# Jarvis73/PEMP

Measured on AMD Instinct MI355X. Metric: episodes/sec (PEMP stage-1 eval step, PASCAL-5i-shaped 1-shot, ResNet-50), higher is better.
Workload: dtype f32

## Files before the change

pemp_amd/csrc/conv_stem_pool.hip:

```cpp
#include "conv_common.h"

namespace pemp {

typedef __attribute__((address_space(3))) void* lptr_t;

namespace {
constexpr int SP_PH = 8, SP_PW = 8;
constexpr int SP_CH = 2 * SP_PH + 1, SP_CW = 2 * SP_PW + 1;
constexpr int SP_IH = 2 * (SP_CH - 1) + 7, SP_IW = 2 * (SP_CW - 1) + 7;
constexpr int SP_ROWS = SP_CH * SP_CW;
constexpr int SP_NW = (SP_ROWS + 31) / 32;
constexpr int SP_TAPS = 49, SP_NK = 7;
constexpr int SP_XQ = SP_IH * SP_IW;
constexpr int SP_XI = (SP_XQ + 63) / 64;
constexpr int SP_BQ = 64 * 12;
constexpr int SP_LDS_OPS = (SP_XI * 64 + 2 * SP_BQ) * 16, SP_LDS_EPI = SP_ROWS * 64 * 4;
constexpr int SP_LDS = SP_LDS_OPS > SP_LDS_EPI ? SP_LDS_OPS : SP_LDS_EPI;
static_assert(SP_NW * 64 <= 1024 && SP_LDS <= 80 * 1024, "two blocks per CU");

__host__ __device__ constexpr int sp_tap_off(int tap) { return (tap / 7) * SP_IW + tap % 7; }
}

__global__ __launch_bounds__(SP_NW * 64) void conv_stem_pool_kernel(ConvArgs a, int Hp, int Wp, int nph, int npw) {
#if defined(__HIP_DEVICE_COMPILE__)
    extern __shared__ __attribute__((aligned(16))) v4f smem[];
    v4f* Xs = smem;
    v4f* Bs = smem + SP_XI * 64;

    const int tid = threadIdx.x;
    const int lane = tid & 63;
    const int wave = __builtin_amdgcn_readfirstlane(tid >> 6);
    const int lr = lane & 31, lh = lane >> 5;

    const int ntn = a.Cout / 64;
    int t = xcd_tile_order(blockIdx.x, gridDim.x);
    const int n0 = (t % ntn) * 64;
    t /= ntn;
    const int pxb = t % npw;
    t /= npw;
    const int pyb = t % nph, img = t / nph;
    const int ph0 = pyb * SP_PH, pw0 = pxb * SP_PW;
    const int cy0 = 2 * ph0 - 1, cx0 = 2 * pw0 - 1;
    const int iy0 = 2 * cy0 - 3, ix0 = 2 * cx0 - 3;

    const __amdgpu_buffer_rsrc_t rx =
        __builtin_amdgcn_make_buffer_rsrc((void*)(a.x + (size_t)img * a.H * a.W * 4), 0, 0x80000000u, 0x00020000);
    const __amdgpu_buffer_rsrc_t rw = __builtin_amdgcn_make_buffer_rsrc((void*)a.w, 0, 0x80000000u, 0x00020000);

    for (int i = wave; i < SP_XI; i += SP_NW) {
        const int q = i * 64 + lane;
        const int py = q / SP_IW, px = q - py * SP_IW;
        const int iy = iy0 + py, ix = ix0 + px;
        const bool ok = q < SP_XQ && (unsigned)iy < (unsigned)a.H && (unsigned)ix < (unsigned)a.W;
        const unsigned vo = ok ? (unsigned)(iy * a.W + ix) * 16u : 0x80000000u;
        __builtin_amdgcn_raw_ptr_buffer_load_lds(rx, (lptr_t)(Xs + i * 64), 16, vo, 0, 0, 0);
    }
#define PEMP_SP_DMA_B(kt_, buf_)                                                                                  \
    for (int i = wave; i < SP_BQ / 64; i += SP_NW) {                                                              \
        const int q = i * 64 + lane, row = q / 12, pos = q - row * 12;                                            \
        const int src = PEMP_SPLIT3_SWZ(row, pos);                                                                \
        const unsigned vo = (unsigned)((n0 + row) * a.Kpad * 6 + src * 16);                                       \
        __builtin_amdgcn_raw_ptr_buffer_load_lds(rw, (lptr_t)(Bs + (buf_) * SP_BQ + i * 64), 16, vo, (kt_) * 192, 0, 0); \
    }
    PEMP_SP_DMA_B(0, 0);

    const int m = wave * 32 + lr;
    const int mc = m < SP_ROWS ? m : 0;
    const int cy = mc / SP_CW, cx = mc - cy * SP_CW;
    const v4f* Ax = Xs + 2 * cy * SP_IW + 2 * cx;
    const v4f* Bw = Bs + lr * 12;
    const int bsw = (lr >> 2) & 3;
    const v4f zero4 = {0.f, 0.f, 0.f, 0.f};

    f32x16 acc[2];
#pragma unroll
    for (int ni = 0; ni < 2; ++ni)
#pragma unroll
        for (int e = 0; e < 16; ++e) acc[ni][e] = 0.f;

#pragma unroll
    for (int kt = 0; kt < SP_NK; ++kt) {
        asm volatile("s_waitcnt vmcnt(0)" ::: "memory");
        __syncthreads();
        if (kt + 1 < SP_NK) PEMP_SP_DMA_B(kt + 1, (kt + 1) & 1);
        const v4f* Bb = Bw + (kt & 1) * SP_BQ;
#pragma unroll
        for (int s = 0; s < 2; ++s) {
            const int tap0 = kt * 8 + s * 4;
            if (tap0 >= SP_TAPS) continue;
            const bool v00 = tap0 < SP_TAPS, v01 = tap0 + 1 < SP_TAPS, v10 = tap0 + 2 < SP_TAPS, v11 = tap0 + 3 < SP_TAPS;
            const int o00 = v00 ? sp_tap_off(tap0) : 0, o01 = v01 ? sp_tap_off(tap0 + 1) : 0;
            const int o10 = v10 ? sp_tap_off(tap0 + 2) : 0, o11 = v11 ? sp_tap_off(tap0 + 3) : 0;
            v4f x0 = Ax[lh ? o10 : o00], x1 = Ax[lh ? o11 : o01];
            if (!(lh ? v10 : v00)) x0 = zero4;
            if (!(lh ? v11 : v01)) x1 = zero4;
            bf16x8 ah, am, al;
            split3_bf16(x0, x1, ah, am, al);
            const int pb = (2 * s + lh) ^ bsw;
#pragma unroll
            for (int ni = 0; ni < 2; ++ni) {
                const bf16x8 bh = __builtin_bit_cast(bf16x8, Bb[ni * 32 * 12 + pb]);
                const bf16x8 bm = __builtin_bit_cast(bf16x8, Bb[ni * 32 * 12 + 4 + pb]);
                const bf16x8 bl = __builtin_bit_cast(bf16x8, Bb[ni * 32 * 12 + 8 + pb]);
                split3_mma6(acc[ni], ah, am, al, bh, bm, bl);
            }
        }
    }
#undef PEMP_SP_DMA_B

    __syncthreads();
    float* Cs = (float*)smem;
    const bool relu = a.flags & PEMP_CONV_RELU;
#pragma unroll
    for (int ni = 0; ni < 2; ++ni) {
        const int n = n0 + ni * 32 + lr;
        const float sc = a.scale ? a.scale[n] : 1.f, sh = a.shift ? a.shift[n] : 0.f;
#pragma unroll
        for (int e = 0; e < 16; ++e) {
            const int row = wave * 32 + (e & 3) + 8 * (e >> 2) + 4 * lh;
            float o = __builtin_fmaf(acc[ni][e], sc, sh);
            if (relu) o = fmaxf(o, 0.f);
            if (row < SP_ROWS) Cs[row * 64 + ni * 32 + lr] = o;
        }
    }
    __syncthreads();
    for (int i = tid; i < SP_PH * SP_PW * 16; i += SP_NW * 64) {
        const int c4 = i & 15, pp = i >> 4;
        const int py = pp / SP_PW, px = pp - py * SP_PW;
        const int ph = ph0 + py, pw = pw0 + px;
        if (ph >= Hp || pw >= Wp) continue;
        v4f mx = {-INFINITY, -INFINITY, -INFINITY, -INFINITY};
#pragma unroll
        for (int dy = 0; dy < 3; ++dy) {
            const int ly = 2 * py + dy;
            if ((unsigned)(cy0 + ly) >= (unsigned)a.Ho) continue;
#pragma unroll
            for (int dx = 0; dx < 3; ++dx) {
                const int lx = 2 * px + dx;
                if ((unsigned)(cx0 + lx) >= (unsigned)a.Wo) continue;
                const v4f v = *(const v4f*)(Cs + (ly * SP_CW + lx) * 64 + c4 * 4);
                mx.x = fmaxf(mx.x, v.x);
                mx.y = fmaxf(mx.y, v.y);
                mx.z = fmaxf(mx.z, v.z);
                mx.w = fmaxf(mx.w, v.w);
            }
        }
        *(v4f*)(a.y + ((size_t)(img * Hp + ph) * Wp + pw) * a.ldy + n0 + c4 * 4) = mx;
    }
#endif
}

int conv_stem_pool_out(int i) {
    int o = (i + 2 - 3 + 1) / 2 + 1;
    if ((o - 1) * 2 >= i + 1) --o;
    return o;
}

int launch_conv_stem_pool(const ConvArgs& a, hipStream_t st) {
    if (!(a.flags & PEMP_CONV_STEM4) || a.KH != 7 || a.KW != 7 || a.stride != 2 || a.pad != 3 || a.dil != 1 || a.Kpad != SP_NK * 32) {
        set_error("conv2d: POOL3S2 needs the 7x7 / stride 2 / pad 3 NHWC4 stem (Kpad %d)", SP_NK * 32);
        return -1;
    }
    if (a.res || a.padv || a.stats || a.rowmask || (a.flags & (PEMP_CONV_SHIFT_PER_IMAGE | PEMP_CONV_BF16_IO))) {
        set_error("conv2d: POOL3S2 takes no residual, padding value, per-image shift or statistics");
        return -1;
    }
    const int Hp = conv_stem_pool_out(a.Ho), Wp = conv_stem_pool_out(a.Wo);
    const int nph = cdiv(Hp, SP_PH), npw = cdiv(Wp, SP_PW);
    const long long grid = (long long)a.N * nph * npw * (a.Cout / 64);
    if ((long long)a.H * a.W * 16 >= (1ll << 31) || (long long)a.Cout * a.Kpad * 6 >= (1ll << 31) || grid >= (1ll << 31) ||
        (long long)a.N * Hp * Wp * a.ldy >= (1ll << 31)) {
        set_error("conv2d: POOL3S2 operands outside 32-bit addressing");
        return -1;
    }
    static_assert(SP_LDS > 64 * 1024, "dynamic LDS attribute");
    hipError_t e = hipFuncSetAttribute((const void*)conv_stem_pool_kernel, hipFuncAttributeMaxDynamicSharedMemorySize, SP_LDS);
    if (e != hipSuccess) {
        set_error("hipFuncSetAttribute(lds=%d): %s", SP_LDS, hipGetErrorString(e));
        return (int)e;
    }
    hipLaunchKernelGGL(conv_stem_pool_kernel, dim3((unsigned)grid), dim3(SP_NW * 64), SP_LDS, st, a, Hp, Wp, nph, npw);
    return launch_status("conv_stem_pool");
}

}
```

scratch/s3_layers_bench.py:

```python
import argparse
import hashlib
import os
import sys

import torch

sys.path.insert(0, os.path.dirname(os.path.dirname(os.path.abspath(__file__))))
from pemp_amd import ops

UNSPLIT = (43, 42, 41, 44, 46, 47, 49)
SPLIT = (52, 51, 54, 56)
PANEL = ops.SPLIT3_PANEL_TILES
PRESPLIT = ops.SPLIT3_PRESPLIT_TILES
RING = getattr(ops, "SPLIT3_RING_TILES", ())
ROW3 = ops.SPLIT3_ROW3_TILES
LAYERS = ((256, 1024, 1, 1, True, False), (512, 1024, 1, 1, False, False), (1024, 256, 1, 1, False, False),
          (256, 256, 3, 2, False, False), (128, 512, 1, 1, True, False), (1024, 512, 1, 1, False, False),
          (256, 256, 3, 2, False, True),
          (64, 256, 1, 1, True, False, 1, 101), (64, 256, 1, 1, False, False, 1, 101), (256, 512, 1, 1, False, False, 2, 101),
          (128, 128, 3, 1, False, False), (128, 128, 3, 1, False, False, 2, 101), (64, 64, 3, 1, False, False, 1, 101),
          (512, 128, 1, 1, False, False),
          (512, 256, 1, 1, False, False), (256, 256, 1, 1, False, False),
          (64, 256, 1, 1, True, False, 1, 51, 101),
          (64, 64, 3, 1, False, False, 2, 101),
          (256, 256, 3, 12, False, True))


def timed(fn, reps, n=5):
    for _ in range(2):
        fn()
    e0, e1 = torch.cuda.Event(enable_timing=True), torch.cuda.Event(enable_timing=True)
    best, worst = 1e9, 0.0
    for _ in range(reps):
        e0.record()
        for _ in range(n):
            fn()
        e1.record()
        e1.synchronize()
        us = e0.elapsed_time(e1) / n * 1e3
        best, worst = min(best, us), max(worst, us)
    return best, worst


def presplit(x):
    h = x.to(torch.bfloat16)
    r = x - h.float()
    m = r.to(torch.bfloat16)
    lo = (r - m.float()).to(torch.bfloat16)
    return torch.stack([p.reshape(*x.shape[:-1], x.shape[-1] // 32, 32) for p in (h, m, lo)], dim=-2).contiguous()


def digest(t):
    return hashlib.sha1(t.cpu().numpy().tobytes()).hexdigest()[:16]


def rs2_row(dev, N, HW, HR, cin, cout, name, keep, reps):
    g = torch.Generator().manual_seed(cin * 7 + cout * 3 + 1001)
    x = torch.randn(N * HW * HW, cin, generator=g).to(dev).view(N, HW, HW, cin)
    w = (torch.randn(cout, cin, 1, 1, generator=g) * (1.0 / cin ** 0.5)).to(dev)
    packed, kpad = ops.pack_conv_weight(w)
    packed = packed.contiguous()
    prm = ops.ConvParams(packed, None, torch.randn(cout, generator=g).to(dev), cin, cout, 1, 1, 1, 0, 1, kpad, False, True, ops.pack_split3(packed))
    res = torch.randn(N, HR, HR, cout, generator=g).to(dev)
    ref = ops.conv2d(x, prm, residual=res[:, ::2, ::2, :].contiguous(), tile=43).clone()
    out = torch.empty_like(ref)
    fl = 2.0 * N * HW * HW * cout * cin
    cells = []
    for tile in keep(ops.res_s2_tiles(prm)):
        run = lambda: ops.conv2d(x, prm, residual=res, residual_stride=2, out=out, tile=tile)
        out.zero_()
        run()
        same = torch.equal(out, ref)
        us, worst = timed(run, reps)
        cells.append(f"{tile}: {us:7.1f}..{worst:6.1f}us {fl / us / 1e6:5.1f}TF{'' if same else ' !'}")
    print(f"{name:>16} k1 d1 res1 | " + " | ".join(cells), flush=True)
    print(f"{'':>16} hash 43={digest(ref)}", flush=True)


def main():
    ap = argparse.ArgumentParser()
    ap.add_argument("--only", default="", help="cin-cout-kK[-padv]: one layer")
    ap.add_argument("--reps", type=int, default=3)
    ap.add_argument("--ids", default="", help="comma-separated tile ids: only these are timed (a counter run of one kernel)")
    ap.add_argument("--producers", action="store_true", help="with --ids: time the selected ids as producers of a pre-split output too")
    ap.add_argument("--res", type=int, choices=(0, 1), default=None, help="run the selected layers without / with a residual, whatever their row says")
    args = ap.parse_args()
    dev = torch.device("cuda:0")
    N = 50
    keep = lambda ids: tuple(t for t in ids if not args.ids or str(t) in args.ids.split(","))
    for layer in LAYERS:
        cin, cout, k, dil, has_res, padv = layer[:6]
        stride, HW = layer[6:8] if len(layer) > 6 else (1, 51)
        RS2 = layer[8] if len(layer) > 8 else 0
        has_res = has_res if args.res is None or RS2 else bool(args.res)
        M = N * HW * HW
        HO = (HW - 1) // stride + 1
        name = f"{cin}-{cout}-k{k}" + (f"-d{dil}" if k == 3 and dil > 2 else "") + ("-padv" if padv else "") + (f"-s{stride}" if stride > 1 else "") + (f"-hw{HW}-res{int(has_res)}" if HW != 51 else "") + ("-rs2" if RS2 else "")
        if args.only and name not in args.only.split(","):
            continue
        if RS2:
            rs2_row(dev, N, HW, RS2, cin, cout, name, keep, args.reps)
            continue
        g = torch.Generator().manual_seed(cin * 7 + cout * 3 + k)
        buf = torch.empty(M + 4, cin, device=dev)
        buf[:M] = torch.randn(M, cin, generator=g).to(dev)
        buf[M:] = torch.randn(cin, generator=g).to(dev)
        x, pv = buf[:M].view(N, HW, HW, cin), buf[M]
        w = (torch.randn(cout, cin, k, k, generator=g) * (1.0 / (cin * k * k) ** 0.5)).to(dev)
        packed, kpad = ops.pack_conv_weight(w)
        packed = packed.contiguous()
        prm = ops.ConvParams(packed, None, torch.randn(cout, generator=g).to(dev), cin, cout, k, k, stride, dil if k == 3 else 0, dil, kpad,
                             False, True, ops.pack_split3(packed))
        res = torch.randn(N, HO, HO, cout, generator=g).to(dev) if has_res else None
        pad_value = pv if padv else None
        out = torch.empty(N, HO, HO, cout, device=dev)
        fl = 2.0 * N * HO * HO * cout * k * k * cin
        ref = ops.conv2d(x, prm, residual=res, pad_value=pad_value, tile=43).clone()
        cells, hashes = [], [f"43={digest(ref)}"]
        panel = PANEL if k == 1 and kpad <= 256 and not padv else ()
        ring = RING if k == 1 and kpad >= 128 and not has_res and not padv and cout % 128 == 0 else ()
        for tile in keep(UNSPLIT + ring + panel + SPLIT):
            if cout % ops._tile_bn(tile):
                continue
            run = lambda: ops.conv2d(x, prm, residual=res, pad_value=pad_value, out=out, tile=tile)
            run()
            same = torch.equal(out, ref)
            if tile in SPLIT:
                hashes.append(f"{tile}=" + ("43" if same else digest(out)))
            us, worst = timed(run, args.reps)
            mark = "" if same else (" ~" if tile in SPLIT else " !")
            cells.append(f"{tile}: {us:7.1f}..{worst:6.1f}us {fl / us / 1e6:5.1f}TF{mark}")
            if tile not in SPLIT and not same:
                hashes.append(f"{tile}=MISMATCH:{digest(out)}")
        if k > 1 and cout % 128 == 0:
            sbuf = torch.zeros((M + 4) * cin * 3, dtype=torch.bfloat16, device=dev)
            sbuf[:(M + 1) * cin * 3] = presplit(buf[:M + 1]).reshape(-1)
            xs, pvs = sbuf[:M * cin * 3].view(N, HW, HW, cin // 32, 3, 32), sbuf[M * cin * 3:(M + 1) * cin * 3].view(cin // 32, 3, 32)
            row3 = ROW3 if k == 3 and stride == 1 and not has_res and not padv and ops.row3_stage_rows(HW, dil) <= ops.ROW3_STAGE_ROWS else ()
            for tile in keep(PRESPLIT + row3):
                run = lambda: ops.conv2d(xs, prm, residual=res, pad_value=pvs if padv else None, out=out, tile=tile, x_split3=True)
                out.zero_()
                run()
                same = torch.equal(out, ref)
                us, worst = timed(run, args.reps)
                cells.append(f"{tile}: {us:7.1f}..{worst:6.1f}us {fl / us / 1e6:5.1f}TF{'' if same else ' !'}")
            if not has_res:
                want = presplit(ref)
                outs = torch.empty_like(want)
                for tile in keep(PRESPLIT):
                    run = lambda: ops.conv2d(xs, prm, pad_value=pvs if padv else None, out=out, tile=tile, x_split3=True, also_split3=outs)
                    out.zero_()
                    run()
                    same = torch.equal(out, ref) and torch.equal(outs.view(torch.int16), want.view(torch.int16))
                    us, worst = timed(run, args.reps)
                    cells.append(f"{tile}+s: {us:7.1f}..{worst:6.1f}us{'' if same else ' !'}")
                del want, outs
            del sbuf, xs, pvs
        if k == 1 and not has_res:
            want = presplit(ref)
            outs = torch.empty_like(want)
            for tile in keep((43, 42, 41, 44, 46, 47, 49) + ring if not args.ids or args.producers else ()):
                if cout % ops._tile_bn(tile):
                    continue
                run = lambda: ops.conv2d(x, prm, out=outs, tile=tile, out_split3=True)
                run()
                same = torch.equal(outs.view(torch.int16), want.view(torch.int16))
                us, worst = timed(run, args.reps)
                cells.append(f"{tile}s: {us:7.1f}..{worst:6.1f}us{'' if same else ' !'}")
            del want, outs
        print(f"{name:>16} k{k} d{dil} res{int(has_res)} | " + " | ".join(cells), flush=True)
        print(f"{'':>16} hash " + " ".join(hashes), flush=True)
    print("(146 / 149 / 246 / 249: on the pre-split input; NNs: id NN writing a pre-split output, ! = not the split of id 43's;")
    print(" NNN+s: id NNN writing fp32 and the pre-split copy, ! = either differs)")
    print("(! = an unsplit id differs from id 43; ~ = a split-K id differs from id 43, expected where it splits)")


if __name__ == "__main__":
    main()
```

Before: 1573.

## Pre-split stem input tile into bf16 planes in LDS with column-parity layout

The fused stem conv+pool kernel now loads the input halo tile into registers, splits each pixel once into three bf16 planes (hi/mid/lo), and stores them in LDS in a layout split by column parity. Previously every MMA step re-ran the fp32-to-3xbf16 split on each tap it read. The parity layout turns the stride-2 tap reads into contiguous 8-byte LDS reads. The cost is synchronous register loads in place of asynchronous buffer-to-LDS DMA, and three plane reads per tap instead of one 16-byte read. A stem benchmark row is also added to the scratch script.

After: 1578, median of 4. About the same (+0.4%).

```diff
diff --git a/pemp_amd/csrc/conv_stem_pool.hip b/pemp_amd/csrc/conv_stem_pool.hip
--- a/pemp_amd/csrc/conv_stem_pool.hip
+++ b/pemp_amd/csrc/conv_stem_pool.hip
@@ -3,6 +3,7 @@
 namespace pemp {
 
 typedef __attribute__((address_space(3))) void* lptr_t;
+typedef __attribute__((ext_vector_type(4))) unsigned int u32x4;
 
 namespace {
 constexpr int SP_PH = 8, SP_PW = 8;
@@ -12,20 +13,24 @@
 constexpr int SP_NW = (SP_ROWS + 31) / 32;
 constexpr int SP_TAPS = 49, SP_NK = 7;
 constexpr int SP_XQ = SP_IH * SP_IW;
-constexpr int SP_XI = (SP_XQ + 63) / 64;
+constexpr int SP_XR = (SP_XQ + SP_NW * 64 - 1) / (SP_NW * 64);
+constexpr int SP_XW2 = (SP_IW + 1) / 2;
+constexpr int SP_XH = SP_IH * SP_XW2, SP_XP = 2 * SP_XH;
 constexpr int SP_BQ = 64 * 12;
-constexpr int SP_LDS_OPS = (SP_XI * 64 + 2 * SP_BQ) * 16, SP_LDS_EPI = SP_ROWS * 64 * 4;
+constexpr int SP_LDS_OPS = 3 * SP_XP * 8 + 2 * SP_BQ * 16, SP_LDS_EPI = SP_ROWS * 64 * 4;
 constexpr int SP_LDS = SP_LDS_OPS > SP_LDS_EPI ? SP_LDS_OPS : SP_LDS_EPI;
 static_assert(SP_NW * 64 <= 1024 && SP_LDS <= 80 * 1024, "two blocks per CU");
-
-__host__ __device__ constexpr int sp_tap_off(int tap) { return (tap / 7) * SP_IW + tap % 7; }
+static_assert((3 * SP_XP * 8) % 16 == 0, "the weight stages are quads");
+
+__host__ __device__ constexpr int sp_pix_off(int py, int px) { return (px & 1) * SP_XH + py * SP_XW2 + (px >> 1); }
+__host__ __device__ constexpr int sp_tap_off(int tap) { return sp_pix_off(tap / 7, tap % 7); }
 }
 
 __global__ __launch_bounds__(SP_NW * 64) void conv_stem_pool_kernel(ConvArgs a, int Hp, int Wp, int nph, int npw) {
 #if defined(__HIP_DEVICE_COMPILE__)
     extern __shared__ __attribute__((aligned(16))) v4f smem[];
-    v4f* Xs = smem;
-    v4f* Bs = smem + SP_XI * 64;
+    u32x2* Xs = (u32x2*)smem;
+    v4f* Bs = smem + 3 * SP_XP * 8 / 16;
 
     const int tid = threadIdx.x;
     const int lane = tid & 63;
@@ -47,13 +52,19 @@
         __builtin_amdgcn_make_buffer_rsrc((void*)(a.x + (size_t)img * a.H * a.W * 4), 0, 0x80000000u, 0x00020000);
     const __amdgpu_buffer_rsrc_t rw = __builtin_amdgcn_make_buffer_rsrc((void*)a.w, 0, 0x80000000u, 0x00020000);
 
-    for (int i = wave; i < SP_XI; i += SP_NW) {
-        const int q = i * 64 + lane;
+    v4f xq[SP_XR + 1];
+    int xd[SP_XR + 1];
+    xq[SP_XR] = v4f{0.f, 0.f, 0.f, 0.f};
+    xd[SP_XR] = -1;
+#pragma unroll
+    for (int r = 0; r < SP_XR; ++r) {
+        const int q = r * SP_NW * 64 + tid;
         const int py = q / SP_IW, px = q - py * SP_IW;
         const int iy = iy0 + py, ix = ix0 + px;
         const bool ok = q < SP_XQ && (unsigned)iy < (unsigned)a.H && (unsigned)ix < (unsigned)a.W;
         const unsigned vo = ok ? (unsigned)(iy * a.W + ix) * 16u : 0x80000000u;
-        __builtin_amdgcn_raw_ptr_buffer_load_lds(rx, (lptr_t)(Xs + i * 64), 16, vo, 0, 0, 0);
+        xq[r] = __builtin_bit_cast(v4f, __builtin_amdgcn_raw_buffer_load_b128(rx, vo, 0, 0));
+        xd[r] = q < SP_XQ ? sp_pix_off(py, px) : -1;
     }
 #define PEMP_SP_DMA_B(kt_, buf_)                                                                                  \
     for (int i = wave; i < SP_BQ / 64; i += SP_NW) {                                                              \
@@ -63,14 +74,30 @@
         __builtin_amdgcn_raw_ptr_buffer_load_lds(rw, (lptr_t)(Bs + (buf_) * SP_BQ + i * 64), 16, vo, (kt_) * 192, 0, 0); \
     }
     PEMP_SP_DMA_B(0, 0);
+#pragma unroll
+    for (int r = 0; r < SP_XR; r += 2) {
+        const int d0 = xd[r], d1 = xd[r + 1];
+        bf16x8 h, m, l;
+        split3_bf16(xq[r], xq[r + 1], h, m, l);
+        const u32x4 hu = __builtin_bit_cast(u32x4, h), mu = __builtin_bit_cast(u32x4, m), lu = __builtin_bit_cast(u32x4, l);
+        if (d0 >= 0) {
+            Xs[d0] = u32x2{hu.x, hu.y};
+            Xs[SP_XP + d0] = u32x2{mu.x, mu.y};
+            Xs[2 * SP_XP + d0] = u32x2{lu.x, lu.y};
+        }
+        if (d1 >= 0) {
+            Xs[d1] = u32x2{hu.z, hu.w};
+            Xs[SP_XP + d1] = u32x2{mu.z, mu.w};
+            Xs[2 * SP_XP + d1] = u32x2{lu.z, lu.w};
+        }
+    }
 
     const int m = wave * 32 + lr;
     const int mc = m < SP_ROWS ? m : 0;
     const int cy = mc / SP_CW, cx = mc - cy * SP_CW;
-    const v4f* Ax = Xs + 2 * cy * SP_IW + 2 * cx;
+    const u32x2* Ax = Xs + sp_pix_off(2 * cy, 2 * cx);
     const v4f* Bw = Bs + lr * 12;
     const int bsw = (lr >> 2) & 3;
-    const v4f zero4 = {0.f, 0.f, 0.f, 0.f};
 
     f32x16 acc[2];
 #pragma unroll
@@ -91,11 +118,18 @@
             const bool v00 = tap0 < SP_TAPS, v01 = tap0 + 1 < SP_TAPS, v10 = tap0 + 2 < SP_TAPS, v11 = tap0 + 3 < SP_TAPS;
             const int o00 = v00 ? sp_tap_off(tap0) : 0, o01 = v01 ? sp_tap_off(tap0 + 1) : 0;
             const int o10 = v10 ? sp_tap_off(tap0 + 2) : 0, o11 = v11 ? sp_tap_off(tap0 + 3) : 0;
-            v4f x0 = Ax[lh ? o10 : o00], x1 = Ax[lh ? o11 : o01];
-            if (!(lh ? v10 : v00)) x0 = zero4;
-            if (!(lh ? v11 : v01)) x1 = zero4;
-            bf16x8 ah, am, al;
-            split3_bf16(x0, x1, ah, am, al);
+            const u32x2* p0 = Ax + (lh ? o10 : o00);
+            const u32x2* p1 = Ax + (lh ? o11 : o01);
+            const bool z0 = !(lh ? v10 : v00), z1 = !(lh ? v11 : v01);
+            bf16x8 af[3];
+#pragma unroll
+            for (int pl = 0; pl < 3; ++pl) {
+                u32x2 f0 = p0[pl * SP_XP], f1 = p1[pl * SP_XP];
+                if (z0) f0 = u32x2{0u, 0u};
+                if (z1) f1 = u32x2{0u, 0u};
+                af[pl] = __builtin_bit_cast(bf16x8, u32x4{f0.x, f0.y, f1.x, f1.y});
+            }
+            const bf16x8 ah = af[0], am = af[1], al = af[2];
             const int pb = (2 * s + lh) ^ bsw;
 #pragma unroll
             for (int ni = 0; ni < 2; ++ni) {
diff --git a/scratch/s3_layers_bench.py b/scratch/s3_layers_bench.py
--- a/scratch/s3_layers_bench.py
+++ b/scratch/s3_layers_bench.py
@@ -77,9 +77,25 @@
     print(f"{'':>16} hash 43={digest(ref)}", flush=True)
 
 
+def stem_row(dev, N, reps):
+    g = torch.Generator().manual_seed(401)
+    x = torch.randn(N, 401, 401, 4, generator=g).to(dev)
+    w = (torch.randn(64, 4, 7, 7, generator=g) / 14.0).to(dev)
+    packed, kpad = ops.pack_conv_weight(w, stem4=True)
+    packed = packed.contiguous()
+    prm = ops.ConvParams(packed, torch.randn(64, generator=g).to(dev), torch.randn(64, generator=g).to(dev), 4, 64, 7, 7, 2, 3, 1, kpad,
+                         True, True, w3pool=ops.pack_split3(packed))
+    out = ops.stem_pool(x, prm).clone()
+    run = lambda: ops.stem_pool(x, prm, out=out)
+    us, worst = timed(run, reps)
+    fl = 2.0 * N * 201 * 201 * 64 * 49 * 4
+    print(f"{'stem':>16} k7 s2 pool | fused: {us:7.1f}..{worst:6.1f}us {fl / us / 1e6:5.1f}TF", flush=True)
+    print(f"{'':>16} hash fused={digest(out)}", flush=True)
+
+
 def main():
     ap = argparse.ArgumentParser()
-    ap.add_argument("--only", default="", help="cin-cout-kK[-padv]: one layer")
+    ap.add_argument("--only", default="", help="cin-cout-kK[-padv]: one layer; stem: the fused stem")
     ap.add_argument("--reps", type=int, default=3)
     ap.add_argument("--ids", default="", help="comma-separated tile ids: only these are timed (a counter run of one kernel)")
     ap.add_argument("--producers", action="store_true", help="with --ids: time the selected ids as producers of a pre-split output too")
@@ -88,6 +104,8 @@
     dev = torch.device("cuda:0")
     N = 50
     keep = lambda ids: tuple(t for t in ids if not args.ids or str(t) in args.ids.split(","))
+    if not args.ids and (not args.only or "stem" in args.only.split(",")):
+        stem_row(dev, N, args.reps)
     for layer in LAYERS:
         cin, cout, k, dil, has_res, padv = layer[:6]
         stride, HW = layer[6:8] if len(layer) > 6 else (1, 51)
```
